# dfm/tinygp

Measured on NVIDIA B200. Metric: log_probability/sec, higher is better.
Workload: dtype f64

## Files before the change

### tinygp_b200/csrc/common.cuh

```cuda
#pragma once
#include <cuda_runtime.h>
#include <stdint.h>
#include <stdio.h>
#include <math.h>
#include <string>
#include <vector>
#include <stdexcept>
#include "../../include/b200gp.h"

#define TILE 128

struct GpError : std::runtime_error {
    using std::runtime_error::runtime_error;
};

#define CUDA_CHECK(expr)                                                                   \
    do {                                                                                   \
        cudaError_t _e = (expr);                                                           \
        if (_e != cudaSuccess) {                                                           \
            char _buf[512];                                                                \
            snprintf(_buf, sizeof(_buf), "%s failed at %s:%d: %s", #expr, __FILE__,        \
                     __LINE__, cudaGetErrorString(_e));                                    \
            throw GpError(_buf);                                                           \
        }                                                                                  \
    } while (0)

struct KProg {
    int n;
    int op[B200GP_PROG_MAX_INSTR];
    int dist[B200GP_PROG_MAX_INSTR];
    double p0[B200GP_PROG_MAX_INSTR];
    double p1[B200GP_PROG_MAX_INSTR];
    int metric[B200GP_PROG_MAX_INSTR];
    int nmetric;
    int mcols;
    int mrows[B200GP_PROG_MAX_METRICS];
    double M[B200GP_PROG_MAX_METRICS][B200GP_METRIC_MAX_DIM * B200GP_METRIC_MAX_DIM];
};

KProg parse_prog(const double* prog, int n_rows, int ndim);

struct CachedBuf {
    void* ptr;
    size_t bytes;
};

struct b200gp_ctx {
    int device = 0;
    cudaStream_t stream = nullptr;
    bool own_stream = false;
    std::string err;
    int64_t launches = 0;
    int64_t nb = 1024;
    bool profile = false;
    b200gp_profile prof{};
    std::vector<CachedBuf> cache;
    cudaEvent_t ev0 = nullptr, ev1 = nullptr;
    int num_sms = 148;
    int64_t peak_iters = 4096;
    int64_t qs_chunk_max = 256;
    int64_t qs_chunk = 0;
    int64_t qsm_chunk = 0;
    int64_t qsm_sequential_redos = 0;
    int64_t qs_tree = 1;
    int64_t potf2_version = 2;
    int64_t qs_kernel = 1;
    int64_t qs_occupancy = 1;
    int64_t build_fast = 2;
    int64_t panel_fused = 0;
    int64_t oz_splitk = 1024;
    int64_t mg_splitk = 0;
    int64_t oz_splitk_force = 0;
    int64_t nb_batched = 4096;
    int64_t oz_slices = 7;
    int64_t oz_lookahead = 0;
    cudaStream_t stream2 = nullptr;
    int64_t build_ahead = 0;
    int64_t panel_overlap = 2;
    cudaStream_t stream3 = nullptr;
    const double* fuse_resid = nullptr;
    int64_t fuse_n = 0;
    double* fuse_y = nullptr;
    double* fuse_x = nullptr;
    int64_t solve_overlap = 1;
    cudaStream_t stream_solve = nullptr;
    int64_t panel_chain = 1;
    cudaStream_t stream_hi = nullptr;
    int64_t oz_prefetch = 0;
    int64_t oz_pairing = 1;
    int64_t oz_layout = 0;
    int64_t oz_cluster = 2;
    int64_t oz_subpanel = 0;
    int64_t oz_l2promo = 3;
    int64_t oz_min_n = 8192;
    struct Pending { cudaEvent_t a, b; double* acc; };
    std::vector<Pending> pending;
    std::vector<cudaEvent_t> event_pool;
    cudaEvent_t get_event();
    void flush_timers();

    void* alloc(size_t bytes);
    void release(void* p, size_t bytes);
    void trim();
};

struct Scratch {
    b200gp_ctx* c;
    size_t bytes;
    void* p;
    Scratch(b200gp_ctx* ctx, size_t nbytes) : c(ctx), bytes(nbytes), p(ctx->alloc(nbytes)) {}
    ~Scratch() { c->release(p, bytes); }
    Scratch(const Scratch&) = delete;
    Scratch& operator=(const Scratch&) = delete;
    double* f64() const { return static_cast<double*>(p); }
};

struct ProfTimer {
    b200gp_ctx* c;
    double* acc;
    cudaEvent_t a = nullptr;
    ProfTimer(b200gp_ctx* ctx, double* field) : c(ctx), acc(field) {
        if (c->profile) {
            a = c->get_event();
            cudaEventRecord(a, c->stream);
        }
    }
    ~ProfTimer() {
        if (c->profile) {
            cudaEvent_t b = c->get_event();
            cudaEventRecord(b, c->stream);
            c->pending.push_back({a, b, acc});
        }
    }
};

#define API_BEGIN(ctxptr)            \
    b200gp_ctx* _ctx = (ctxptr);     \
    if (!_ctx) return 1;             \
    try {                            \
        CUDA_CHECK(cudaSetDevice(_ctx->device));
#define API_END                      \
        return 0;                    \
    } catch (const std::exception& e) { \
        _ctx->err = e.what();        \
        return 2;                    \
    }

struct b200gp_dense {
    b200gp_ctx* ctx = nullptr;
    int64_t n = 0;
    int64_t np = 0;
    int64_t ld = 0;
    size_t mat_bytes = 0;
    double* mat_alloc = nullptr;
    double* mat = nullptr;
    double* linv = nullptr;
    int* info_dev = nullptr;
    int info = 0;
    bool has_prog = false;
    KProg prog{};
    int ndim = 0;
    double* X_dev = nullptr;
    double* diag_dev = nullptr;
    bool owns_inputs = false;
};

void dense_build_rect(b200gp_ctx* ctx, const KProg& prog, const double* X1, int64_t n1,
                      const double* X2, int64_t n2, int ndim, const double* diag_or_null,
                      double* out, int64_t ld, int64_t rows_pad, int64_t cols_pad);
void dense_conditioned_covariance_to_host(b200gp_ctx* ctx, const KProg& P, const double* At, int64_t mp, int64_t kp,
                                          const double* xt_dev, const double* dt_dev, int nd, int64_t m,
                                          double* out_host);
b200gp_dense* dense_factor_from_prog(b200gp_ctx* ctx, const KProg& prog, const double* X_dev,
                                     int64_t n, int ndim, const double* diag_dev, bool copy_inputs);
void dense_factor_inplace(b200gp_dense* s, bool generate);
void dense_destroy(b200gp_dense* s);
double dense_logdet_half(b200gp_dense* s);
void dense_solve_vec_dev(b200gp_dense* s, double* y_dev , double* x_dev ,
                         bool transpose);
double dense_sumsq_dev(b200gp_ctx* ctx, const double* x_dev, int64_t n);
```

### tinygp_b200/csrc/dense.cu

```cuda
#include "common.cuh"
#include <limits.h>

#include "kprog.cuh"

KProg parse_prog(const double* prog, int n_rows, int ndim) { return parse_prog_impl(prog, n_rows, ndim); }

struct BuildArgs {
    const double* X1;
    const double* X2;
    const double* diag;
    double* out;
    int64_t ld;
    int64_t n1, n2;
    int64_t rows_pad, cols_pad;
    int64_t row_off, col_off;
    int ndim;
    int pad_identity;
    const KProg* progs;
    int64_t batch_stride;
    const double* batch_consts;
    int batch_op, batch_l2;
    int lower_only;
};

// ... 407 lines not shown
        CUDA_CHECK(cudaFuncSetAttribute(gemm_nt_kernel<true>, cudaFuncAttributeMaxDynamicSharedMemorySize, SMEM_BYTES));
        CUDA_CHECK(cudaFuncSetAttribute(gemm_nt_kernel<false>, cudaFuncAttributeMaxDynamicSharedMemorySize, SMEM_BYTES));
        g_attr_set = true;
    }
    int64_t ntiles;
    if (g.lower)
        ntiles = (int64_t)g.tiles_m * (g.tiles_m + 1) / 2;
    else
        ntiles = (int64_t)g.tiles_m * g.tiles_n;
    if (ntiles <= 0) return;
    dim3 grid((unsigned)ntiles, (unsigned)(g.batch > 0 ? g.batch : 1));
    if (g.lower)
        gemm_nt_kernel<true><<<grid, THREADS, SMEM_BYTES, ctx->stream>>>(P, g);
    else
        gemm_nt_kernel<false><<<grid, THREADS, SMEM_BYTES, ctx->stream>>>(P, g);
    CUDA_CHECK(cudaGetLastError());
    ctx->launches++;
}
}

static const KProg& empty_prog() {
    static KProg p{};
    return p;
}

static void gemm_nt(b200gp_ctx* ctx, double* C, int64_t ldc, const double* A, int64_t lda,
                    const double* B, int64_t ldb, int tiles_m, int tiles_n, int K, double alpha,
                    int beta_mode, int lower, int batch = 1, int64_t strideA = 0, int64_t strideB = 0,
                    int64_t strideC = 0) {
    gemm::Args g{};
    g.A = A; g.lda = lda; g.B = B; g.ldb = ldb; g.C = C; g.ldc = ldc;
    g.tiles_m = tiles_m; g.tiles_n = tiles_n; g.K = K; g.alpha = alpha;
    g.beta_mode = beta_mode; g.lower = lower;
    g.batch = batch; g.strideA = strideA; g.strideB = strideB; g.strideC = strideC;
    gemm::launch(ctx, empty_prog(), g);
}

#define PF_LD 129
#define PF_THREADS 512
constexpr int PF_SMEM = (TILE * PF_LD + 4 * TILE + TILE) * (int)sizeof(double);

__global__ void __launch_bounds__(PF_THREADS, 1) potf2_trtri_kernel(double* A, int64_t lda, double* linv,
                                                                    int* info, int global_off, int64_t strideA,
                                                                    int64_t stride_linv) {
    extern __shared__ __align__(16) double sm[];
    A += (int64_t)blockIdx.x * strideA;
    linv += (int64_t)blockIdx.x * stride_linv;
    info += blockIdx.x;
    double* S = sm;
    double* red = sm + TILE * PF_LD;
    double* tmp = red + 4 * TILE;
    const int tid = threadIdx.x;
    const int i = tid & (TILE - 1);
    const int part = tid >> 7;

    for (int e = tid; e < TILE * TILE; e += PF_THREADS) {
        const int r = e >> 7, c = e & (TILE - 1);
        S[r * PF_LD + c] = (c <= r) ? A[(int64_t)r * lda + c] : 0.0;
    }
    __syncthreads();

    for (int j = 0; j < TILE; ++j) {
        double s = 0.0;
        const double ajj = S[j * PF_LD + j];
        const double aij = S[i * PF_LD + j];
        if (i >= j) {
            const double* ri = S + i * PF_LD;
            const double* rj = S + j * PF_LD;
            for (int k = part; k < j; k += 4) s += ri[k] * rj[k];
        }
        red[part * TILE + i] = s;
        __syncthreads();
        if (part == 0 && i >= j) {
            const double vj = ajj - (red[j] + red[TILE + j] + red[2 * TILE + j] + red[3 * TILE + j]);
            if (i == j) {
                if (!(vj > 0.0)) atomicMin(info, global_off + j + 1);
                S[j * PF_LD + j] = sqrt(vj);
            } else {
                const double vi = aij - (red[i] + red[TILE + i] + red[2 * TILE + i] + red[3 * TILE + i]);
                S[i * PF_LD + j] = vi / sqrt(vj);
            }
        }
        __syncthreads();
    }

    for (int e = tid; e < TILE * TILE; e += PF_THREADS) {
        const int r = e >> 7, c = e & (TILE - 1);
        if (c <= r) A[(int64_t)r * lda + c] = S[r * PF_LD + c];
    }
    __syncthreads();

    for (int j = TILE - 1; j >= 0; --j) {
        if (tid < TILE) tmp[tid] = S[tid * PF_LD + j];
        __syncthreads();
        const double dj = 1.0 / tmp[j];
        double s = 0.0;
        if (i > j) {
            const double* ri = S + i * PF_LD;
            for (int k = j + 1 + part; k <= i; k += 4) s += ri[k] * tmp[k];
        }
        red[part * TILE + i] = s;
        __syncthreads();
        if (part == 0) {
            if (i == j)
                S[j * PF_LD + j] = dj;
            else if (i > j)
                S[i * PF_LD + j] = -dj * (red[i] + red[TILE + i] + red[2 * TILE + i] + red[3 * TILE + i]);
        }
        __syncthreads();
    }
    for (int e = tid; e < TILE * TILE; e += PF_THREADS) {
        const int r = e >> 7, c = e & (TILE - 1);
        linv[e] = (c <= r) ? S[r * PF_LD + c] : 0.0;
    }
}

constexpr int PF2_SMEM = (TILE * PF_LD + TILE * 8 + 4 * TILE * 8) * (int)sizeof(double);

__global__ void __launch_bounds__(PF_THREADS, 1) potf2_trtri_kernel_v2(double* A, int64_t lda, double* linv, int* info,
                                                                       int global_off, int64_t strideA,
                                                                       int64_t stride_linv) {
    extern __shared__ __align__(16) double sm[];
    A += (int64_t)blockIdx.x * strideA;
    linv += (int64_t)blockIdx.x * stride_linv;
    info += blockIdx.x;
    double* S = sm;
    double* T = sm + TILE * PF_LD;
    double* red = T + TILE * 8;
    const int tid = threadIdx.x;
    const int i = tid & (TILE - 1);
    const int part = tid >> 7;

    for (int e = tid; e < TILE * TILE; e += PF_THREADS) {
        const int r = e >> 7, c = e & (TILE - 1);
        S[r * PF_LD + c] = (c <= r) ? A[(int64_t)r * lda + c] : 0.0;
    }
    __syncthreads();

    for (int jb = 0; jb < TILE / 8; ++jb) {
        const int j0 = jb * 8;
        const bool owner = (tid < TILE && tid >= j0);
        double D[8][8], arow[8];
        if (owner) {
#pragma unroll
            for (int a = 0; a < 8; ++a)
#pragma unroll
                for (int b = 0; b <= a; ++b) D[a][b] = S[(j0 + a) * PF_LD + j0 + b];
#pragma unroll
            for (int c = 0; c < 8; ++c) arow[c] = S[tid * PF_LD + j0 + c];
        }
        __syncthreads();
        if (owner) {
            const int r = tid;
            int firstbad = -1;
            double invd[8];
#pragma unroll
            for (int c = 0; c < 8; ++c) {
                double v = D[c][c];
#pragma unroll
                for (int k = 0; k < c; ++k) v -= D[c][k] * D[c][k];
                if (!(v > 0.0) && firstbad < 0) firstbad = c;
                const double sq = sqrt(v);
                const double isq = 1.0 / sq;
                D[c][c] = sq;
                invd[c] = isq;
#pragma unroll
                for (int a = c + 1; a < 8; ++a) {
                    double w = D[a][c];
#pragma unroll
                    for (int k = 0; k < c; ++k) w -= D[a][k] * D[c][k];
                    D[a][c] = w * isq;
                }
            }
            if (r == j0 && firstbad >= 0) atomicMin(info, global_off + j0 + firstbad + 1);
            if (r < j0 + 8) {
                if (r == j0) {
#pragma unroll
                    for (int a = 0; a < 8; ++a)
#pragma unroll
                        for (int b = 0; b <= a; ++b) S[(j0 + a) * PF_LD + j0 + b] = D[a][b];
                }
            } else {
                double x[8];
#pragma unroll
                for (int c = 0; c < 8; ++c) {
                    double w = arow[c];
#pragma unroll
                    for (int k = 0; k < c; ++k) w -= x[k] * D[c][k];
                    x[c] = w * invd[c];
                }
#pragma unroll
                for (int c = 0; c < 8; ++c) S[r * PF_LD + j0 + c] = x[c];
            }
        }
        __syncthreads();
        const int m = TILE - j0 - 8;
        if (m > 0) {
            const int nt = m >> 2, ntiles = nt * (nt + 1) / 2;
            for (int e = tid; e < ntiles; e += PF_THREADS) {
                int ti = (int)((sqrt(8.0 * (double)e + 1.0) - 1.0) * 0.5);
                while ((ti + 1) * (ti + 2) / 2 <= e) ++ti;
                while (ti * (ti + 1) / 2 > e) --ti;
                const int tj = e - ti * (ti + 1) / 2;
                const int i0 = j0 + 8 + 4 * ti, c0 = j0 + 8 + 4 * tj;
                double acc[4][4];
#pragma unroll
                for (int a = 0; a < 4; ++a)
#pragma unroll
                    for (int b = 0; b < 4; ++b) acc[a][b] = 0.0;
#pragma unroll
                for (int k = 0; k < 8; ++k) {
                    double lr[4], lc[4];
#pragma unroll
                    for (int a = 0; a < 4; ++a) {
                        lr[a] = S[(i0 + a) * PF_LD + j0 + k];
                        lc[a] = S[(c0 + a) * PF_LD + j0 + k];
                    }
#pragma unroll
                    for (int a = 0; a < 4; ++a)
#pragma unroll
                        for (int b = 0; b < 4; ++b) acc[a][b] += lr[a] * lc[b];
                }
#pragma unroll
                for (int a = 0; a < 4; ++a)
#pragma unroll
                    for (int b = 0; b < 4; ++b)
                        if (c0 + b <= i0 + a) S[(i0 + a) * PF_LD + c0 + b] -= acc[a][b];
            }
        }
        __syncthreads();
    }

    for (int e = tid; e < TILE * TILE; e += PF_THREADS) {
        const int r = e >> 7, c = e & (TILE - 1);
        if (c <= r) A[(int64_t)r * lda + c] = S[r * PF_LD + c];
    }
    __syncthreads();

    for (int jb = TILE / 8 - 1; jb >= 0; --jb) {
        const int j0 = jb * 8;
        for (int e = tid; e < TILE * 8; e += PF_THREADS) {
            const int k = e >> 3, c = e & 7;
            T[e] = (k >= j0) ? S[k * PF_LD + j0 + c] : 0.0;
        }
        __syncthreads();
        double acc[8];
#pragma unroll
        for (int c = 0; c < 8; ++c) acc[c] = 0.0;
        if (i >= j0 + 8) {
            const double* ri = S + i * PF_LD;
            for (int k = j0 + 8 + part; k <= i; k += 4) {
                const double xik = ri[k];
#pragma unroll
                for (int c = 0; c < 8; ++c) acc[c] += xik * T[k * 8 + c];
            }
        }
#pragma unroll
        for (int c = 0; c < 8; ++c) red[(part * TILE + i) * 8 + c] = acc[c];
        __syncthreads();
        if (part == 0 && i >= j0) {
            double Di[8][8], rd[8];
#pragma unroll
            for (int c = 0; c < 8; ++c) rd[c] = 1.0 / T[(j0 + c) * 8 + c];
#pragma unroll
            for (int c = 0; c < 8; ++c) {
                Di[c][c] = rd[c];
#pragma unroll
                for (int a = c + 1; a < 8; ++a) {
                    double w = 0.0;
#pragma unroll
                    for (int k = c; k < a; ++k) w += T[(j0 + a) * 8 + k] * Di[k][c];
                    Di[a][c] = -w * rd[a];
                }
            }
            if (i < j0 + 8) {
                if (i == j0) {
#pragma unroll
                    for (int a = 0; a < 8; ++a)
#pragma unroll
                        for (int c = 0; c <= a; ++c) S[(j0 + a) * PF_LD + j0 + c] = Di[a][c];
                }
            } else {
                double v[8];
#pragma unroll
                for (int c = 0; c < 8; ++c)
                    v[c] = red[i * 8 + c] + red[(TILE + i) * 8 + c] + red[(2 * TILE + i) * 8 + c] + red[(3 * TILE + i) * 8 + c];
#pragma unroll
                for (int c = 0; c < 8; ++c) {
                    double w = 0.0;
#pragma unroll
                    for (int cp = c; cp < 8; ++cp) w += v[cp] * Di[cp][c];
                    S[i * PF_LD + j0 + c] = -w;
                }
            }
        }
        __syncthreads();
    }
    for (int e = tid; e < TILE * TILE; e += PF_THREADS) {
        const int r = e >> 7, c = e & (TILE - 1);
        linv[e] = (c <= r) ? S[r * PF_LD + c] : 0.0;
    }
}

static void potf2(b200gp_ctx* ctx, double* A, int64_t lda, double* linv, int* info, int global_off, int batch = 1,
                  int64_t strideA = 0, int64_t stride_linv = 0) {
    static bool attr = false;
    if (!attr) {
        CUDA_CHECK(cudaFuncSetAttribute(potf2_trtri_kernel, cudaFuncAttributeMaxDynamicSharedMemorySize, PF_SMEM));
        attr = true;
    }
    if (ctx->potf2_version == 1) {
        potf2_trtri_kernel<<<batch, PF_THREADS, PF_SMEM, ctx->stream>>>(A, lda, linv, info, global_off, strideA, stride_linv);
    } else {
        static bool attr2 = false;
        if (!attr2) {
            CUDA_CHECK(cudaFuncSetAttribute(potf2_trtri_kernel_v2, cudaFuncAttributeMaxDynamicSharedMemorySize, PF2_SMEM));
            attr2 = true;
        }
        potf2_trtri_kernel_v2<<<batch, PF_THREADS, PF2_SMEM, ctx->stream>>>(A, lda, linv, info, global_off, strideA,
                                                                          stride_linv);
    }
    CUDA_CHECK(cudaGetLastError());
    ctx->launches++;
}

__global__ void set_int_kernel(int* p, int v) { *p = v; }

static void dense_panel_factor_lookahead(b200gp_dense* s, int64_t k0, int64_t kb, int64_t lo = -1, int64_t hi = -1);

void dense_panel_factor(b200gp_dense* s, int64_t k0, int64_t kb) {
    b200gp_ctx* ctx = s->ctx;
    const int64_t np = s->np, ld = s->ld;
    double* M = s->mat;
    if (ctx->panel_overlap == 2 && kb > TILE) {
        dense_panel_factor_lookahead(s, k0, kb);
        return;
    }
    const bool overlap = ctx->panel_overlap == 1;
    cudaStream_t main_stream = ctx->stream;
    cudaEvent_t e_main = nullptr, e_side = nullptr;
    if (overlap) {
        if (!ctx->stream3) CUDA_CHECK(cudaStreamCreateWithFlags(&ctx->stream3, cudaStreamNonBlocking));
        e_main = ctx->get_event();
        e_side = ctx->get_event();
    }
    for (int64_t j0 = 0; j0 < kb; j0 += TILE) {
        const int64_t c0 = k0 + j0;
        const int rows_below = (int)((np - c0) / TILE) - 1;
        bool side_pending = false;
        if (j0 > 0) {
            if (overlap && rows_below > 0) {
                CUDA_CHECK(cudaEventRecord(e_main, main_stream));
                CUDA_CHECK(cudaStreamWaitEvent(ctx->stream3, e_main, 0));
                ctx->stream = ctx->stream3;
                try {
                    gemm_nt(ctx, M + (c0 + TILE) * ld + c0, ld, M + (c0 + TILE) * ld + k0, ld, M + c0 * ld + k0, ld,
                            rows_below, 1, (int)j0, -1.0, 1, 0);
                } catch (...) {
                    ctx->stream = main_stream;
                    throw;
                }
                ctx->stream = main_stream;
                CUDA_CHECK(cudaEventRecord(e_side, ctx->stream3));
                side_pending = true;
                gemm_nt(ctx, M + c0 * ld + c0, ld, M + c0 * ld + k0, ld, M + c0 * ld + k0, ld, 1, 1, (int)j0, -1.0, 1, 0);
            } else {
                gemm_nt(ctx, M + c0 * ld + c0, ld, M + c0 * ld + k0, ld, M + c0 * ld + k0, ld,
                        (int)((np - c0) / TILE), 1, (int)j0, -1.0, 1, 0);
            }
        }
        potf2(ctx, M + c0 * ld + c0, ld, s->linv + (c0 / TILE) * TILE * TILE, s->info_dev, (int)c0);
        if (c0 + TILE < np) {
            if (side_pending) CUDA_CHECK(cudaStreamWaitEvent(main_stream, e_side, 0));
            gemm_nt(ctx, M + (c0 + TILE) * ld + c0, ld, M + (c0 + TILE) * ld + c0, ld,
                    s->linv + (c0 / TILE) * TILE * TILE, TILE, (int)((np - c0 - TILE) / TILE), 1, TILE,
                    1.0, 0, 0);
        }
    }
    if (overlap) {
        ctx->event_pool.push_back(e_main);
        ctx->event_pool.push_back(e_side);
    }
}

static void dense_panel_factor_lookahead(b200gp_dense* s, int64_t k0, int64_t kb, int64_t lo, int64_t hi) {
    b200gp_ctx* ctx = s->ctx;
    const int64_t np = s->np, ld = s->ld;
    double* M = s->mat;
    const int64_t bend = k0 + kb;
    if (lo < 0) { lo = bend; hi = np; }
    const int own = (hi > lo) ? (int)((hi - lo) / TILE) : 0;
    cudaStream_t wide = ctx->stream;
    if (!ctx->stream_hi) {
        int lo = 0, hi = 0;
        CUDA_CHECK(cudaDeviceGetStreamPriorityRange(&lo, &hi));
        CUDA_CHECK(cudaStreamCreateWithPriority(&ctx->stream_hi, cudaStreamNonBlocking, hi));
    }
    cudaStream_t chain = ctx->stream_hi;
    cudaEvent_t ev = ctx->get_event();
    struct Restore { b200gp_ctx* c; cudaStream_t st; ~Restore() { c->stream = st; } } restore{ctx, wide};
    CUDA_CHECK(cudaEventRecord(ev, wide));
    CUDA_CHECK(cudaStreamWaitEvent(chain, ev, 0));
    const bool chain_right = (ctx->panel_chain == 1);
    for (int64_t j0 = 0; j0 < kb; j0 += TILE) {
        const int64_t c0 = k0 + j0;
        const int blk = (int)((bend - c0) / TILE);
        const double* li = s->linv + (c0 / TILE) * TILE * TILE;
        ctx->stream = chain;
        if (j0 > 0 && !chain_right)
            gemm_nt(ctx, M + c0 * ld + c0, ld, M + c0 * ld + k0, ld, M + c0 * ld + k0, ld, blk, 1, (int)j0, -1.0, 1, 0);
        potf2(ctx, M + c0 * ld + c0, ld, s->linv + (c0 / TILE) * TILE * TILE, s->info_dev, (int)c0);
        if (own) CUDA_CHECK(cudaEventRecord(ev, chain));
        if (blk > 1) gemm_nt(ctx, M + (c0 + TILE) * ld + c0, ld, M + (c0 + TILE) * ld + c0, ld, li, TILE, blk - 1, 1, TILE, 1.0, 0, 0);
        if (chain_right && blk > 1)
            gemm_nt(ctx, M + (c0 + TILE) * ld + (c0 + TILE), ld, M + (c0 + TILE) * ld + c0, ld, M + (c0 + TILE) * ld + c0, ld,
                    blk - 1, blk - 1, TILE, -1.0, 1, 1);
        if (own) {
            CUDA_CHECK(cudaStreamWaitEvent(wide, ev, 0));
            ctx->stream = wide;
            if (j0 > 0) gemm_nt(ctx, M + lo * ld + c0, ld, M + lo * ld + k0, ld, M + c0 * ld + k0, ld, own, 1, (int)j0, -1.0, 1, 0);
            gemm_nt(ctx, M + lo * ld + c0, ld, M + lo * ld + c0, ld, li, TILE, own, 1, TILE, 1.0, 0, 0);
        }
    }
    ctx->stream = wide;
    CUDA_CHECK(cudaEventRecord(ev, chain));
    CUDA_CHECK(cudaStreamWaitEvent(wide, ev, 0));
    ctx->event_pool.push_back(ev);
}

void dense_panel_factor_rows(b200gp_dense* s, int64_t k0, int64_t kb, int64_t r0, int64_t r1) {
    b200gp_ctx* ctx = s->ctx;
    const int64_t np = s->np, ld = s->ld;
    double* M = s->mat;
    const int64_t bend = k0 + kb;
    int64_t lo = (r0 > bend) ? r0 : bend, hi = (r1 < np) ? r1 : np;
    if (lo % TILE || hi % TILE) throw GpError("panel_factor_rows: row range must be 128-aligned");
    if (ctx->panel_overlap == 2 && kb > TILE) {
        dense_panel_factor_lookahead(s, k0, kb, lo, (hi > lo) ? hi : lo);
        return;
    }
    const int own = (hi > lo) ? (int)((hi - lo) / TILE) : 0;
    for (int64_t j0 = 0; j0 < kb; j0 += TILE) {
        const int64_t c0 = k0 + j0;
        const int blk = (int)((bend - c0) / TILE);
        if (j0 > 0) {
            gemm_nt(ctx, M + c0 * ld + c0, ld, M + c0 * ld + k0, ld, M + c0 * ld + k0, ld, blk, 1, (int)j0, -1.0, 1, 0);
            if (own) gemm_nt(ctx, M + lo * ld + c0, ld, M + lo * ld + k0, ld, M + c0 * ld + k0, ld, own, 1, (int)j0, -1.0, 1, 0);
        }
        potf2(ctx, M + c0 * ld + c0, ld, s->linv + (c0 / TILE) * TILE * TILE, s->info_dev, (int)c0);
        const double* li = s->linv + (c0 / TILE) * TILE * TILE;
        if (blk > 1) gemm_nt(ctx, M + (c0 + TILE) * ld + c0, ld, M + (c0 + TILE) * ld + c0, ld, li, TILE, blk - 1, 1, TILE, 1.0, 0, 0);
        if (own) gemm_nt(ctx, M + lo * ld + c0, ld, M + lo * ld + c0, ld, li, TILE, own, 1, TILE, 1.0, 0, 0);
    }
}

void dense_build_region(b200gp_dense* s, int64_t r0, int64_t c0, int64_t ncols) {
    b200gp_ctx* ctx = s->ctx;
    const int64_t np = s->np, ld = s->np;
    BuildArgs a{};
    a.X1 = s->X_dev + r0 * s->ndim;
    a.X2 = s->X_dev + c0 * s->ndim;
    a.diag = s->diag_dev; a.out = s->mat + r0 * ld + c0; a.ld = ld;
    a.n1 = (s->n > r0) ? (s->n - r0) : 0;
    a.n2 = (s->n > c0) ? ((s->n - c0 < ncols) ? (s->n - c0) : ncols) : 0;
    a.rows_pad = np - r0; a.cols_pad = ncols;
    a.row_off = r0; a.col_off = c0; a.ndim = s->ndim; a.pad_identity = 1;
    dim3 grid((unsigned)((ncols + BUILD_COLS - 1) / BUILD_COLS), (unsigned)((np - r0 + BUILD_ROWS - 1) / BUILD_ROWS));
    ProfTimer t(ctx, &ctx->prof.build_ms);
    launch_build_rect(ctx, grid, s->prog, a);
    CUDA_CHECK(cudaGetLastError());
    ctx->launches++;
    ctx->prof.build_bytes += 8.0 * (double)(np - r0) * (double)ncols;
}

double dense_kernel_diag_value(const KProg& P) { return kprog_eval_zero(P); }

struct BuildRegionArgs { int64_t r0, r1, c0, ncols; };
void dense_build_rows(b200gp_dense* s, const BuildRegionArgs& q) {
    b200gp_ctx* ctx = s->ctx;
    const int64_t ld = s->ld;
    BuildArgs a{};
    a.X1 = s->X_dev + q.r0 * s->ndim;
    a.X2 = s->X_dev + q.c0 * s->ndim;
    a.diag = s->diag_dev; a.out = s->mat + q.r0 * ld + q.c0; a.ld = ld;
    a.n1 = (s->n > q.r0) ? ((s->n - q.r0 < q.r1 - q.r0) ? (s->n - q.r0) : (q.r1 - q.r0)) : 0;
    a.n2 = (s->n > q.c0) ? ((s->n - q.c0 < q.ncols) ? (s->n - q.c0) : q.ncols) : 0;
    a.rows_pad = q.r1 - q.r0; a.cols_pad = q.ncols;
    a.row_off = q.r0; a.col_off = q.c0; a.ndim = s->ndim; a.pad_identity = 1;
    dim3 grid((unsigned)((q.ncols + BUILD_COLS - 1) / BUILD_COLS), (unsigned)((q.r1 - q.r0 + BUILD_ROWS - 1) / BUILD_ROWS));
    ProfTimer t(ctx, &ctx->prof.build_ms);
    launch_build_rect(ctx, grid, s->prog, a);
    CUDA_CHECK(cudaGetLastError());
    ctx->launches++;
    ctx->prof.build_bytes += 8.0 * (double)(q.r1 - q.r0) * (double)q.ncols;
}

void dense_factor_ozaki(b200gp_dense* s, int S);

void dense_factor_inplace(b200gp_dense* s, bool generate) {
    b200gp_ctx* ctx = s->ctx;
    const int64_t np = s->np, ld = s->np;
    int64_t NB = ctx->nb;
    if (NB < TILE) NB = TILE;
    NB = (NB / TILE) * TILE;
    double* M = s->mat;

    if (generate && ctx->oz_slices > 0 && np >= ctx->oz_min_n) {
        dense_factor_ozaki(s, (int)ctx->oz_slices);
        return;
    }

    set_int_kernel<<<1, 1, 0, ctx->stream>>>(s->info_dev, INT_MAX);
    ctx->launches++;

    if (generate) {
        dense_build_region(s, 0, 0, (NB < np) ? NB : np);
    }

    for (int64_t k0 = 0; k0 < np; k0 += NB) {
        const int64_t kb = (NB < np - k0) ? NB : (np - k0);
        {
            ProfTimer t(ctx, &ctx->prof.panel_ms);
            dense_panel_factor(s, k0, kb);
        }
        const int64_t r0 = k0 + kb;
        if (r0 < np) {
            gemm::Args g{};
            g.A = M + r0 * ld + k0; g.lda = ld;
            g.B = M + r0 * ld + k0; g.ldb = ld;
            g.C = M + r0 * ld + r0; g.ldc = ld;
            g.tiles_m = g.tiles_n = (int)((np - r0) / TILE);
            g.K = (int)kb; g.alpha = -1.0; g.lower = 1;
            g.beta_mode = (generate && k0 == 0) ? 2 : 1;
            g.X = s->X_dev; g.diag = s->diag_dev; g.ndim = s->ndim; g.n_valid = s->n;
            g.row0 = r0; g.col0 = r0;
            ProfTimer t(ctx, &ctx->prof.syrk_ms);
            gemm::launch(ctx, (g.beta_mode == 2) ? s->prog : empty_prog(), g);
            const double T = (double)g.tiles_m;
            ctx->prof.syrk_flop += T * (T + 1.0) / 2.0 * 2.0 * TILE * TILE * (double)kb;
            ctx->prof.syrk_launches++;
        }
    }
    CUDA_CHECK(cudaMemcpyAsync(&s->info, s->info_dev, sizeof(int), cudaMemcpyDeviceToHost, ctx->stream));
    CUDA_CHECK(cudaStreamSynchronize(ctx->stream));
    if (s->info == INT_MAX) s->info = 0;
    if (s->info > s->n) s->info = 0;
}

__global__ void __launch_bounds__(1024) reduce_kernel(const double* v, int64_t stride, int64_t n, int mode, double* out,
                                                      int64_t batch_stride) {
    __shared__ double sh[1024];
    v += (int64_t)blockIdx.x * batch_stride;
    out += blockIdx.x;
    double acc = 0.0;
    for (int64_t i = threadIdx.x; i < n; i += 1024) {
        const double x = v[i * stride];
        acc += (mode == 0) ? log(x) : x * x;
    }
    sh[threadIdx.x] = acc;
    __syncthreads();
    for (int o = 512; o > 0; o >>= 1) {
        if ((int)threadIdx.x < o) sh[threadIdx.x] += sh[threadIdx.x + o];
        __syncthreads();
    }
    if (threadIdx.x == 0) out[0] = sh[0];
}

static double reduce_to_host(b200gp_ctx* ctx, const double* v, int64_t stride, int64_t n, int mode) {
    double* d = (double*)ctx->alloc(sizeof(double));
    reduce_kernel<<<1, 1024, 0, ctx->stream>>>(v, stride, n, mode, d, 0);
    CUDA_CHECK(cudaGetLastError());
    ctx->launches++;
    double h = 0.0;
    CUDA_CHECK(cudaMemcpyAsync(&h, d, sizeof(double), cudaMemcpyDeviceToHost, ctx->stream));
    CUDA_CHECK(cudaStreamSynchronize(ctx->stream));
    ctx->release(d, sizeof(double));
    return h;
}

double dense_logdet_half(b200gp_dense* s) { return reduce_to_host(s->ctx, s->mat, s->np + 1, s->n, 0); }
double dense_sumsq_dev(b200gp_ctx* ctx, const double* x_dev, int64_t n) { return reduce_to_host(ctx, x_dev, 1, n, 1); }

__global__ void __launch_bounds__(256) trsv_fwd_step(const double* __restrict__ mat, int64_t ld,
                                                      const double* __restrict__ linv_j, double* y, double* x,
                                                      int j, int64_t np, int64_t stride_mat, int64_t stride_linv) {
    __shared__ __align__(32) double ys[TILE];
    __shared__ __align__(32) double xs[TILE];
    const int tid = threadIdx.x, warp = tid >> 5, lane = tid & 31;
    mat += (int64_t)blockIdx.y * stride_mat;
    linv_j += (int64_t)blockIdx.y * stride_linv;
    y += (int64_t)blockIdx.y * np;
    x += (int64_t)blockIdx.y * np;
    if (tid < TILE) ys[tid] = y[(int64_t)j * TILE + tid];
    __syncthreads();
    for (int r = warp; r < TILE; r += 8) {
        const double* row = linv_j + r * TILE;
        double s = 0.0;
        for (int c = lane; c <= r; c += 32) s += row[c] * ys[c];
        for (int o = 16; o > 0; o >>= 1) s += __shfl_xor_sync(0xffffffffu, s, o);
        if (lane == 0) xs[r] = s;
    }
    __syncthreads();
    if (blockIdx.x == 0 && tid < TILE) x[(int64_t)j * TILE + tid] = xs[tid];
    const int64_t rbase = (int64_t)(j + 1) * TILE + (int64_t)blockIdx.x * 64 + warp * 8;
    const double4 xv = *reinterpret_cast<const double4*>(xs + lane * 4);
#pragma unroll
    for (int rr = 0; rr < 8; ++rr) {
        const int64_t r = rbase + rr;
        if (r >= np) break;
        const double4 lv = *reinterpret_cast<const double4*>(mat + r * ld + (int64_t)j * TILE + lane * 4);
        double s = lv.x * xv.x + lv.y * xv.y + lv.z * xv.z + lv.w * xv.w;
        for (int o = 16; o > 0; o >>= 1) s += __shfl_xor_sync(0xffffffffu, s, o);
        if (lane == 0) y[r] -= s;
    }
}
// ... 726 lines not shown
```

Measured before the change: 1.147.

## Add DMMA-based blocked potf2+trtri kernel for 128x128 diagonal tiles

```diff
diff --git a/tinygp_b200/csrc/common.cuh b/tinygp_b200/csrc/common.cuh
--- a/tinygp_b200/csrc/common.cuh
+++ b/tinygp_b200/csrc/common.cuh
@@ -63,7 +63,7 @@
     int64_t qsm_chunk = 0;
     int64_t qsm_sequential_redos = 0;
     int64_t qs_tree = 1;
-    int64_t potf2_version = 2;
+    int64_t potf2_version = 3;
     int64_t qs_kernel = 1;
     int64_t qs_occupancy = 1;
     int64_t build_fast = 2;
diff --git a/tinygp_b200/csrc/dense.cu b/tinygp_b200/csrc/dense.cu
--- a/tinygp_b200/csrc/dense.cu
+++ b/tinygp_b200/csrc/dense.cu
@@ -733,6 +733,187 @@
     }
 }
 
+namespace pf3 {
+constexpr int THREADS = 256;
+constexpr int LD = 132;
+constexpr int LDD = 20;
+constexpr int LDT = 68;
+constexpr int SMEM = (TILE * LD + 8 * 16 * LDD + 64 * LDT) * (int)sizeof(double);
+
+__device__ __forceinline__ void tile16(double (&acc)[2][2][2], const double* A, int ars, int acs, const double* B,
+                                       int brs, int bcs, int k0, int k1, double sign) {
+    const int lane = threadIdx.x & 31, g = lane >> 2, t = lane & 3;
+#pragma unroll 4
+    for (int k = k0 + t; k < k1; k += 4) {
+        const double a0 = sign * A[g * ars + k * acs], a1 = sign * A[(g + 8) * ars + k * acs];
+        const double b0 = B[g * brs + k * bcs], b1 = B[(g + 8) * brs + k * bcs];
+        gemm::dmma884(acc[0][0][0], acc[0][0][1], a0, b0);
+        gemm::dmma884(acc[0][1][0], acc[0][1][1], a0, b1);
+        gemm::dmma884(acc[1][0][0], acc[1][0][1], a1, b0);
+        gemm::dmma884(acc[1][1][0], acc[1][1][1], a1, b1);
+    }
+}
+__device__ __forceinline__ void zero16(double (&acc)[2][2][2]) {
+#pragma unroll
+    for (int i = 0; i < 8; ++i) (&acc[0][0][0])[i] = 0.0;
+}
+__device__ __forceinline__ void load16(double (&acc)[2][2][2], const double* C, int ldc) {
+    const int lane = threadIdx.x & 31, g = lane >> 2, t = lane & 3;
+#pragma unroll
+    for (int i = 0; i < 2; ++i)
+#pragma unroll
+        for (int j = 0; j < 2; ++j)
+#pragma unroll
+            for (int v = 0; v < 2; ++v) acc[i][j][v] = C[(8 * i + g) * ldc + 8 * j + 2 * t + v];
+}
+__device__ __forceinline__ void store16(const double (&acc)[2][2][2], double* C, int ldc, bool lower) {
+    const int lane = threadIdx.x & 31, g = lane >> 2, t = lane & 3;
+#pragma unroll
+    for (int i = 0; i < 2; ++i)
+#pragma unroll
+        for (int j = 0; j < 2; ++j)
+#pragma unroll
+            for (int v = 0; v < 2; ++v) {
+                const int r = 8 * i + g, c = 8 * j + 2 * t + v;
+                if (!lower || c <= r) C[r * ldc + c] = acc[i][j][v];
+            }
+}
+
+template <int C>
+__device__ __forceinline__ void leaf_col(double (&a)[16], double (&rinv)[16], int l, int& bad) {
+    const double d = __shfl_sync(0xffffffffu, a[C], C);
+    if (!(d > 0.0) && bad < 0) bad = C;
+    const double r = rsqrt(d);
+    rinv[C] = r;
+    const double lc = (l == C) ? d * r : a[C] * r;
+    a[C] = lc;
+#pragma unroll
+    for (int j = C + 1; j < 16; ++j) {
+        const double ljc = __shfl_sync(0xffffffffu, lc, j);
+        if (l >= j) a[j] = fma(-lc, ljc, a[j]);
+    }
+    if constexpr (C + 1 < 16) leaf_col<C + 1>(a, rinv, l, bad);
+}
+template <int K>
+__device__ __forceinline__ void leaf_inv_row(const double* D, double (&x)[16], double (&s)[16], const double (&rinv)[16],
+                                             int l) {
+    x[K] = (K < l) ? 0.0 : (K == l ? rinv[K] : -s[K] * rinv[K]);
+#pragma unroll
+    for (int i = K + 1; i < 16; ++i) s[i] = fma(D[i * LD + K], x[K], s[i]);
+    if constexpr (K + 1 < 16) leaf_inv_row<K + 1>(D, x, s, rinv, l);
+}
+
+__device__ __forceinline__ void leaf16(double* D, double* Di, int* info, int goff) {
+    const int lane = threadIdx.x & 31, l = lane & 15;
+    double a[16], rinv[16];
+#pragma unroll
+    for (int c = 0; c < 16; ++c) a[c] = (c <= l) ? D[l * LD + c] : 0.0;
+    int bad = -1;
+    leaf_col<0>(a, rinv, l, bad);
+    if (lane == 0 && bad >= 0) atomicMin(info, goff + bad + 1);
+    if (lane < 16) {
+#pragma unroll
+        for (int c = 0; c < 16; ++c)
+            if (c <= l) D[l * LD + c] = a[c];
+    }
+    __syncwarp();
+    double x[16], s[16];
+#pragma unroll
+    for (int k = 0; k < 16; ++k) s[k] = 0.0;
+    leaf_inv_row<0>(D, x, s, rinv, l);
+    if (lane < 16) {
+#pragma unroll
+        for (int k = 0; k < 16; ++k) Di[k * LDD + l] = x[k];
+    }
+}
+}
+
+__global__ void __launch_bounds__(pf3::THREADS, 1) potf2_trtri_kernel_v3(double* A, int64_t lda, double* linv, int* info,
+                                                                         int global_off, int64_t strideA,
+                                                                         int64_t stride_linv) {
+    using namespace pf3;
+    extern __shared__ __align__(16) double sm[];
+    A += (int64_t)blockIdx.x * strideA;
+    linv += (int64_t)blockIdx.x * stride_linv;
+    info += blockIdx.x;
+    double* S = sm;
+    double* Di = S + TILE * LD;
+    double* T = Di + 8 * 16 * LDD;
+    const int tid = threadIdx.x, warp = tid >> 5;
+
+#pragma unroll 8
+    for (int e = tid; e < TILE * TILE; e += THREADS) {
+        const int r = e >> 7, c = e & (TILE - 1);
+        S[r * LD + c] = (c <= r) ? A[(int64_t)r * lda + c] : 0.0;
+    }
+    __syncthreads();
+
+    for (int kb = 0; kb < 8; ++kb) {
+        const int k0 = 16 * kb, r0 = k0 + 16, nt = 7 - kb;
+        if (warp == 0) leaf16(S + k0 * LD + k0, Di + kb * 16 * LDD, info, global_off + k0);
+        __syncthreads();
+        if (nt == 0) break;
+        if (warp < nt) {
+            double acc[2][2][2];
+            zero16(acc);
+            double* P = S + (r0 + 16 * warp) * LD + k0;
+            tile16(acc, P, LD, 1, Di + kb * 16 * LDD, LDD, 1, 0, 16, 1.0);
+            __syncwarp();
+            store16(acc, P, LD, false);
+        }
+        __syncthreads();
+        for (int e = warp; e < nt * (nt + 1) / 2; e += THREADS / 32) {
+            int ti = 0;
+            while ((ti + 1) * (ti + 2) / 2 <= e) ++ti;
+            const int tj = e - ti * (ti + 1) / 2;
+            double acc[2][2][2];
+            double* C = S + (r0 + 16 * ti) * LD + r0 + 16 * tj;
+            load16(acc, C, LD);
+            tile16(acc, S + (r0 + 16 * ti) * LD + k0, LD, 1, S + (r0 + 16 * tj) * LD + k0, LD, 1, 0, 16, -1.0);
+            store16(acc, C, LD, ti == tj);
+        }
+        __syncthreads();
+    }
+
+#pragma unroll 8
+    for (int e = tid; e < TILE * TILE; e += THREADS) {
+        const int r = e >> 7, c = e & (TILE - 1);
+        if (c <= r) A[(int64_t)r * lda + c] = S[r * LD + c];
+    }
+    __syncthreads();
+    for (int e = tid; e < 8 * 256; e += THREADS) {
+        const int kb = e >> 8, i = (e >> 4) & 15, c = e & 15;
+        S[(16 * kb + i) * LD + 16 * kb + c] = Di[kb * 16 * LDD + i * LDD + c];
+    }
+    __syncthreads();
+
+    for (int s = 16; s < TILE; s *= 2) {
+        const int nb = s / 16, ntile = (TILE / (2 * s)) * nb * nb;
+        for (int e = warp; e < ntile; e += THREADS / 32) {
+            const int p = e / (nb * nb), ti = (e / nb) % nb, tj = e % nb, o = 2 * s * p;
+            double acc[2][2][2];
+            zero16(acc);
+            tile16(acc, S + (o + s + 16 * ti) * LD + o, LD, 1, S + o * LD + o + 16 * tj, 1, LD, 16 * tj, s, 1.0);
+            store16(acc, T + (p * s + 16 * ti) * LDT + 16 * tj, LDT, false);
+        }
+        __syncthreads();
+        for (int e = warp; e < ntile; e += THREADS / 32) {
+            const int p = e / (nb * nb), ti = (e / nb) % nb, tj = e % nb, o = 2 * s * p;
+            double acc[2][2][2];
+            zero16(acc);
+            tile16(acc, S + (o + s + 16 * ti) * LD + o + s, LD, 1, T + p * s * LDT + 16 * tj, 1, LDT, 0, 16 * ti + 16,
+                   -1.0);
+            store16(acc, S + (o + s + 16 * ti) * LD + o + 16 * tj, LD, false);
+        }
+        __syncthreads();
+    }
+#pragma unroll 8
+    for (int e = tid; e < TILE * TILE; e += THREADS) {
+        const int r = e >> 7, c = e & (TILE - 1);
+        linv[e] = (c <= r) ? S[r * LD + c] : 0.0;
+    }
+}
+
 static void potf2(b200gp_ctx* ctx, double* A, int64_t lda, double* linv, int* info, int global_off, int batch = 1,
                   int64_t strideA = 0, int64_t stride_linv = 0) {
     static bool attr = false;
@@ -742,6 +923,14 @@
     }
     if (ctx->potf2_version == 1) {
         potf2_trtri_kernel<<<batch, PF_THREADS, PF_SMEM, ctx->stream>>>(A, lda, linv, info, global_off, strideA, stride_linv);
+    } else if (ctx->potf2_version == 3) {
+        static bool attr3 = false;
+        if (!attr3) {
+            CUDA_CHECK(cudaFuncSetAttribute(potf2_trtri_kernel_v3, cudaFuncAttributeMaxDynamicSharedMemorySize, pf3::SMEM));
+            attr3 = true;
+        }
+        potf2_trtri_kernel_v3<<<batch, pf3::THREADS, pf3::SMEM, ctx->stream>>>(A, lda, linv, info, global_off, strideA,
+                                                                               stride_linv);
     } else {
         static bool attr2 = false;
         if (!attr2) {
```

After: 1.158 (median of 6 runs). +1.0%, better.
